# hkust-vgd/pointwise

Measured on AMD Instinct MI355X. Metric: conv3p fwd+bwd Mpoints/s, higher is better.
Workload: dtype f32; 1 GPU; cfg2 ModelNet40-shaped: B=32 clouds/GPU x N=2048, pointcnn2_acsd conv3p stack 3->9 s1, 9->9 s2, 9->9 s3, 9->9 s4 (+SELU), forward+backward, a different batch every step, next batch's neighbour search enqueued on a side stream under the current backward; global_batch=32, points_per_cloud=2048, parallelism=dp1, backward_kernel_choice=hint from Conv3pStack.tune() at set-up: short lists

## Files before the change

pointwise_amd/csrc/conv3p_abi_search.hpp:

```cpp
namespace {

template <typename T> int run_prep(const T *points, const Call<T> &c)
{
    if (c.skip_prep) {
        if (c.evicted_hinted)
            return hipMemsetAsync(c.L.slot[c.slot].cursor, 0, sizeof(uint32_t) * 2 * (size_t)c.d.B, c.s) == hipSuccess
                       ? CONV3P_OK : CONV3P_ERR_LAUNCH;
        return CONV3P_OK;
    }
    const Dims &d = c.d;
    Scope sc(K_PREP, c.s);
    if (d.N <= 16384 && d.N > kTile) {
        int npad = 128;
        while (npad < d.N) npad <<= 1;
        const int threads = npad / 2 < 1024 ? (npad / 2 < 64 ? 64 : npad / 2) : 1024;
        const size_t lds = (size_t)npad * 8 + 256;
        auto launch = [&](auto kern) {
            launch_lds(kern, dim3(d.B), dim3(threads), lds, c.s, points, d.N, d.ntiles, npad, c.L.pts, c.L.boxes, c.cc);
        };
        switch (npad / threads) {
        case 2: launch(prep_sort_kernel<T, 2>); break;
        case 4: launch(prep_sort_kernel<T, 4>); break;
        case 8: launch(prep_sort_kernel<T, 8>); break;
        default: launch(prep_sort_kernel<T, 16>); break;
        }
        return hip_ok();
    }
    dim3 grid((d.ntiles + kWavesPerBlock - 1) / kWavesPerBlock, d.B);
    hipLaunchKernelGGL(prep_kernel<T>, grid, dim3(256), 0, c.s, points, d.N, d.ntiles, c.L.pts, c.L.boxes, c.cc);
    return hip_ok();
}

template <typename T> size_t search_lds_bytes(const Stencil<T> &st, int gtiles)
{
    return lds_common(st) + a16((size_t)st.ntap * kCntStride * 4) + a16(sizeof(CentreRec<T>) * 64) + 64 * 3 * 4 +
           a16((size_t)gtiles * 64 * 8) + a16((size_t)gtiles * 4) + 32 + kWavesPerBlock * 64 * 4 +
           a16((size_t)kWavesPerBlock * 192 * 4) + a16((size_t)kWavesPerBlock * 256 * 4) + 1024;
}

template <typename T> int run_cloud_min(const T *points, const Call<T> &c)
{
    if (!c.st.window) return CONV3P_OK;
    hipLaunchKernelGGL(cloud_min_kernel<T>, dim3((unsigned)c.d.B), dim3(256), 0, c.s, points, c.d.N, c.L.cmin);
    return hip_ok();
}

template <typename SlotT> inline const uint32_t *sched_of(const SlotT &S)
{
#ifdef CONV3P_DEV_NO_SCHED
    return nullptr;
#else
    return S.sched;
#endif
}

constexpr unsigned long long kShortListsPerPoint = 35, kShortListsPerPointFused = 48;
template <typename T> SchedJob make_sched_job(const Call<T> &c, int slot, bool fused)
{
    const auto &S = c.L.slot[slot];
    return SchedJob{S.segs, S.sched, S.cursor, S.regime,
                    (fused ? kShortListsPerPointFused : kShortListsPerPoint) * (unsigned long long)c.d.B * (unsigned long long)c.d.N};
}

#ifndef CONV3P_DEV_FUSED_M
#define CONV3P_DEV_FUSED_M 6
#endif
template <typename T> bool fused_ok(const Call<T> &c)
{
#ifdef CONV3P_DEV_NO_FUSED_SEARCH
    return false;
#endif
    const Stencil<T> &st = c.st;
    if (c.L.ftab == nullptr || st.window) return false;
    for (int a = 0; a < 3; ++a)
        if (st.ext[a] > kFMaxExt) return false;
    return true;
}
template <typename T> FusedJob<T> make_fused_job(const Call<T> &c)
{
    const auto &S = c.L.slot[c.slot];
    FusedJob<T> j;
    j.st = c.st;
    j.cc = c.cc;
    j.count = S.count;
    j.tcount = S.tcount;
    j.pairs = S.pairs;
    j.segs = S.segs;
    j.qsegs = S.qsegs;
    j.qbm = S.qbm;
    j.qbm_hi = S.qbm_hi;
    for (int a = 0; a < 3; ++a)
        for (int k = 0; k < kFMaxExt; ++k)
            j.clo[a][k] = (float)(((double)k * c.st.step[a] - (double)c.st.full[a] * 0.5) * (double)kFR);
    return j;
}
inline int fused_mask_depth(int elem, int ntiles, int ntap_max, int maxfull_max)
{
    const int mmax = (ntiles + kWavesPerBlock - 1) / kWavesPerBlock;
    int M = std::min(mmax, (int)CONV3P_DEV_FUSED_M);
    if (ntiles <= 32) M = 1;
    if (M < 1) M = 1;
    while (M > 1 && fused_lds(ntap_max, maxfull_max, elem, M).total > 40 * 1024) --M;
    return fused_lds(ntap_max, maxfull_max, elem, M).total > kMaxLds ? 0 : M;
}
template <typename T> int launch_fused(const Call<T> &c, const FusedJobs<T> &jobs, const SchedJobs &sjobs, int njobs, bool schedule = true)
{
    const Dims &d = c.d;
    const BlockMap bm = make_blockmap(d);
    int ntap_max = 1, maxfull_max = 1;
    for (int k = 0; k < njobs; ++k) {
        ntap_max = std::max(ntap_max, jobs.job[k].st.ntap);
        maxfull_max = std::max(maxfull_max, jobs.job[k].st.maxfull);
    }
    const int M = fused_mask_depth((int)sizeof(T), d.ntiles, ntap_max, maxfull_max);
    if (M == 0) return CONV3P_ERR_UNSUPPORTED;
#ifdef CONV3P_DEV_FUSED_LDS_KB
    const size_t lds = std::max(fused_lds(ntap_max, maxfull_max, (int)sizeof(T), M).total, (size_t)CONV3P_DEV_FUSED_LDS_KB * 1024);
#else
    const size_t lds = fused_lds(ntap_max, maxfull_max, (int)sizeof(T), M).total;
#endif
    if (lds > kMaxLds) return CONV3P_ERR_UNSUPPORTED;
    const float inv16 = (float)((double)kFR / (double)c.st.voxel);
    Scope sc(K_SEARCH, c.s);
    hipLaunchKernelGGL(tile_tables_kernel<T>, dim3((d.ntiles + kWavesPerBlock - 1) / kWavesPerBlock, d.B), dim3(256), 0, c.s,
                       c.L.pts, d.ntiles, inv16, c.L.ftab, c.cc.version, c.L.tab_version, c.L.tab_ticket, c.L.tab_inv, c.cc.force);
    bool ext3 = true;
    for (int k = 0; k < njobs; ++k)
        for (int a = 0; a < 3; ++a) ext3 &= jobs.job[k].st.ext[a] == 3;
    auto launch = [&](auto kern) {
        launch_lds(kern, dim3(grid_of(bm), njobs), dim3(256), lds, c.s, c.L.pts, c.L.boxes, c.L.ftab, d.N, d.ntiles, c.L.ngroups, bm,
                   jobs, M, inv16);
    };
    if (ext3) launch(search_fused_kernel<T, true>);
    else launch(search_fused_kernel<T, false>);
#ifndef CONV3P_DEV_NO_SCHED
    if (schedule)
        hipLaunchKernelGGL(tile_sched_kernel, dim3(8, njobs), dim3(1024), 0, c.s, sjobs, d.B, d.ntiles, c.L.ngroups, bm.rounds * d.ntiles);
#endif
    return hip_ok();
}

template <typename T> int add_companions(const Call<T> &c, FusedJobs<T> &fj, SchedJobs &sj, int n)
{
    if (c.cache_key == nullptr || c.skip_prep) return n;
    const CacheRef ref = find_cache(c.cache_key);
    if (!ref) return n;
    CacheHost &h = *ref;
    for (int sl = 0; sl < h.nslots && n < kFusedMaxJobs; ++sl) {
        if (sl == c.slot || h.tags[sl] == 0ull) continue;
        const CacheHost::SlotDesc &sd = h.desc[sl];
        if (sd.voxel != (double)c.st.voxel) continue;
        Dims d2 = c.d;
        d2.fz = sd.fz; d2.fy = sd.fy; d2.fx = sd.fx;
        d2.ntap = sd.fz * sd.fy * sd.fx;
        Call<T> c2;
        c2.d = d2;
        c2.st = make_stencil<T>(d2, sd.stride, c.st.voxel);
        c2.L = c.L;
        c2.slot = sl;
        c2.s = c.s;
        c2.cc = make_ctl(c.L, sl, h.tags[sl], c.cc.epoch, 0);
        if (!fused_ok(c2)) continue;
        if (fused_mask_depth((int)sizeof(T), c.d.ntiles, std::max(c.st.ntap, c2.st.ntap), std::max(c.st.maxfull, c2.st.maxfull)) <
            fused_mask_depth((int)sizeof(T), c.d.ntiles, c.st.ntap, c.st.maxfull))
            continue;
        fj.job[n] = make_fused_job(c2);
        sj.job[n] = make_sched_job(c, sl, true);
        ++n;
    }
    return n;
}
template <typename T> void note_companions_built(const Call<T> &c, const FusedJobs<T> &fj, int n)
{
    if (c.cache_key == nullptr || n <= 1) return;
    const CacheRef ref = find_cache(c.cache_key);
    if (!ref) return;
    CacheHost &h = *ref;
    for (int k = 1; k < n; ++k)
        for (int sl = 0; sl < h.nslots; ++sl)
            if (sl != c.slot && h.tags[sl] == fj.job[k].cc.tag) h.built_gen[sl] = h.gen;
}

template <typename T> int run_search(const Call<T> &c, int32_t *count, bool with_pairs)
{
    if (c.skip_search && with_pairs) return CONV3P_OK;
    const Dims &d = c.d;
    const Stencil<T> &st = c.st;
    const auto &S = c.L.slot[c.slot];
    if (fused_ok(c) && fused_mask_depth((int)sizeof(T), d.ntiles, st.ntap, st.maxfull) > 0 && (!with_pairs || count == S.count)) {
        FusedJobs<T> fj;
        SchedJobs sj;
        fj.job[0] = make_fused_job(c);
        sj.job[0] = make_sched_job(c, c.slot, true);
        if (!with_pairs) {
            FusedJob<T> &j = fj.job[0];
            j.count = count;
            j.tcount = nullptr;
            j.pairs = nullptr;
            j.segs = nullptr;
            j.qsegs = nullptr;
            j.qbm = nullptr;
            j.qbm_hi = nullptr;
            return launch_fused<T>(c, fj, sj, 1, false);
        }
        const int nj = add_companions<T>(c, fj, sj, 1);
        TRY(launch_fused<T>(c, fj, sj, nj));
        note_companions_built<T>(c, fj, nj);
        return CONV3P_OK;
    }
    const size_t lds = search_lds_bytes(st, c.L.gtiles);
    if (lds > kMaxLds) return CONV3P_ERR_UNSUPPORTED;
    const BlockMap bm = make_blockmap(d);
    {
        Scope sc(K_SEARCH, c.s);
        auto launch = [&](auto kern, const T *cmin) {
            launch_lds(kern, dim3(grid_of(bm)), dim3(256), lds, c.s, c.L.pts, c.L.boxes, st, d.N, d.ntiles, c.L.gtiles, c.L.ngroups,
                       bm, count, with_pairs ? S.pairs : nullptr, c.cc, S.segs, S.qsegs, cmin, with_pairs ? S.tcount : nullptr,
                       with_pairs ? S.qbm : nullptr, with_pairs ? S.qbm_hi : nullptr);
        };
        if (st.window) launch(search_kernel<T, true>, c.L.cmin);
        else launch(search_kernel<T, false>, static_cast<const T *>(nullptr));
        if (with_pairs) {
            SchedJobs sj;
            sj.job[0] = make_sched_job(c, c.slot, false);
            hipLaunchKernelGGL(tile_sched_kernel, dim3(8, 1), dim3(1024), 0, c.s, sj, d.B, d.ntiles, c.L.ngroups, bm.rounds * d.ntiles);
        }
    }
    return hip_ok();
}

template <typename T> int run_geometry(const T *points, const Call<T> &c)
{
    TRY(run_prep<T>(points, c));
    TRY(run_cloud_min<T>(points, c));
    return run_search<T>(c, c.L.slot[c.slot].count, true);
}

#ifdef CONV3P_DEV_WALK_STATS
__global__ void walk_stats_kernel(const uint2 *qsegs, const PairEntry *pairs, int ntiles_all, unsigned long long *out)
{
    const int t = blockIdx.x * blockDim.x + threadIdx.x;
    if (t >= ntiles_all) return;
    uint32_t len[64];
    unsigned long long recs = 0, live = 0;
    for (int c = 0; c < 64; ++c) {
        const uint2 sg = qsegs[(size_t)t * 64 + c];
        len[c] = sg.y == kSegOverflow ? 0u : sg.y;
        recs += len[c];
        for (uint32_t i = 0; i < len[c]; ++i) live += code_fwd(pairs[sg.x + i].code) != kNoTap ? 1u : 0u;
    }
    unsigned long long cur = 0, pslw = 0, ideal = 0, curmax = 0, pslmax = 0, idealmax = 0;
    for (int w = 0; w < 4; ++w) {
        uint32_t mx = 0, sum = 0;
        for (int c = 0; c < 16; ++c) { mx = max(mx, len[16 * w + c]); sum += len[16 * w + c]; }
        const unsigned long long a = (mx + 3) / 4;
        uint32_t S = max(1u, (sum + 63) / 64);
        for (;; ++S) {
            uint32_t need = 0;
            for (int c = 0; c < 16; ++c) need += (len[16 * w + c] + S - 1) / S;
            if (need <= 64) break;
        }
        const unsigned long long idl = (sum + 63) / 64;
        cur += a; pslw += S; ideal += idl;
        curmax = max(curmax, a); pslmax = max(pslmax, (unsigned long long)S); idealmax = max(idealmax, idl);
    }
    uint32_t St = max(1u, (uint32_t)((recs + 255) / 256));
    for (;; ++St) {
        uint32_t need = 0;
        for (int c = 0; c < 64; ++c) need += (len[c] + St - 1) / St;
        if (need <= 256) break;
    }
    atomicAdd(&out[0], recs); atomicAdd(&out[1], live); atomicAdd(&out[2], cur); atomicAdd(&out[3], pslw);
    atomicAdd(&out[4], 4ull * St); atomicAdd(&out[5], ideal);
    atomicMax(&out[6], curmax); atomicMax(&out[7], pslmax); atomicMax(&out[8], (unsigned long long)St); atomicMax(&out[9], idealmax);
}
template <typename T> void dev_walk_stats(const Call<T> &c, const char *what, int ci, int co)
{
    const auto &S = c.L.slot[c.slot];
    if (c.L.ngroups != 1) return;
    unsigned long long *d = nullptr, h[10];
    if (hipMalloc(&d, sizeof(h)) != hipSuccess) return;
    (void)hipMemsetAsync(d, 0, sizeof(h), c.s);
    const int nt = c.d.B * c.d.ntiles;
    hipLaunchKernelGGL(walk_stats_kernel, dim3((nt + 63) / 64), dim3(64), 0, c.s, S.qsegs, S.pairs, nt, d);
    (void)hipStreamSynchronize(c.s);
    (void)hipMemcpy(h, d, sizeof(h), hipMemcpyDeviceToHost);
    (void)hipFree(d);
    const double r = (double)h[0];
    fprintf(stderr, "walk_stats %s<%d,%d> stride %d B=%d N=%d: records/point %.2f (true pairs %.2f) | lane use: shipped %.3f (true-pair %.3f), "
            "per-wave proportional %.3f, per-workgroup proportional %.3f, bound %.3f | steps of the slowest wave: shipped %llu, "
            "per-wave prop. %llu, per-wg prop. %llu, bound %llu | mean steps per wave: %.2f / %.2f / %.2f / %.2f\n",
            what, ci, co, c.st.step[0], c.d.B, c.d.N, r / ((double)c.d.B * c.d.N), (double)h[1] / ((double)c.d.B * c.d.N),
            r / (64.0 * h[2]), (double)h[1] / (64.0 * h[2]), r / (64.0 * h[3]), r / (64.0 * h[4]), r / (64.0 * h[5]),
            h[6], h[7], h[8], h[9], h[2] / (4.0 * nt), h[3] / (4.0 * nt), h[4] / (4.0 * nt), h[5] / (4.0 * nt));
}
#endif

template <typename T>
int prepare_multi_impl(const T *points, const int32_t *strides, int K, T voxel, int B, int N, int fz, int fy,
                       int fx, Where wh, void *stream)
{
    if (K <= 0 || K > kMaxJobs || !strides) return CONV3P_ERR_INVALID_ARGUMENT;
    Dims d{B, N, 0, 0, fz, fy, fx, 0, 0};
    for (int k = 0; k < K; ++k) TRY(check(d, strides + 3 * k, (double)voxel, false));
    if ((size_t)B * N == 0) return CONV3P_OK;
    if (!points) return CONV3P_ERR_INVALID_ARGUMENT;
    if (K > wh.nslots) return CONV3P_ERR_WORKSPACE;
    hipStream_t s = static_cast<hipStream_t>(stream);
    SearchJobs<T> jobs;
    FusedJobs<T> fjobs;
    SchedJobs sjobs, fsjobs;
    int njobs = 0, nfused = 0;
    size_t lds = 0;
    bool any_window = false;
    Call<T> c;
    for (int k = 0; k < K; ++k) {
        TRY(begin_call<T>(c, d, strides + 3 * k, voxel, 0, wh, s));
        TRY(run_prep<T>(points, c));
        wh.flags |= CONV3P_CACHE_POINTS_UNCHANGED;
        if (c.skip_search) continue;
        const Stencil<T> &st = c.st;
        const auto &S = c.L.slot[c.slot];
        TRY(run_cloud_min<T>(points, c));
        if (fused_ok(c) && fused_mask_depth((int)sizeof(T), c.d.ntiles, c.st.ntap, c.st.maxfull) > 0) {
            fjobs.job[nfused] = make_fused_job(c);
            fsjobs.job[nfused++] = make_sched_job(c, c.slot, true);
            continue;
        }
        any_window |= st.window != 0;
        const size_t l = search_lds_bytes(st, c.L.gtiles);
        if (l > kMaxLds) return CONV3P_ERR_UNSUPPORTED;
        lds = l > lds ? l : lds;
        SearchJob<T> &j = jobs.job[njobs++];
        j.st = st;
        j.cc = c.cc;
        j.count = S.count;
        j.tcount = S.tcount;
        j.pairs = S.pairs;
        j.segs = S.segs;
        j.qsegs = S.qsegs;
        j.qbm = S.qbm;
        j.qbm_hi = S.qbm_hi;
        sjobs.job[njobs - 1] = make_sched_job(c, c.slot, true);
    }
    if (nfused > 0) TRY(launch_fused<T>(c, fjobs, fsjobs, nfused));
    if (njobs == 0) return CONV3P_OK;
    for (int k = 0; k < njobs; ++k)
        sjobs.job[k].limit = kShortListsPerPoint * (unsigned long long)c.d.B * (unsigned long long)c.d.N;
#ifndef CONV3P_DEV_JOBS_IN_ORDER
    for (int a = 1; a < njobs; ++a)
        for (int b2 = a; b2 > 0; --b2) {
            auto vol = [](const SearchJob<T> &j) { return (long long)j.st.step[0] * j.st.step[1] * j.st.step[2]; };
            if (vol(jobs.job[b2]) <= vol(jobs.job[b2 - 1])) break;
            std::swap(jobs.job[b2], jobs.job[b2 - 1]);
            std::swap(sjobs.job[b2], sjobs.job[b2 - 1]);
        }
#endif
    const BlockMap bm = make_blockmap(c.d);
    {
        Scope sc(K_SEARCH, s);
        auto launch = [&](auto kern) {
            launch_lds(kern, dim3(grid_of(bm), njobs), dim3(256), lds, s, c.L.pts, c.L.boxes, c.d.N, c.d.ntiles, c.L.gtiles,
                       c.L.ngroups, bm, jobs, c.L.cmin);
        };
        if (any_window) launch(search_multi_kernel<T, true>);
        else launch(search_multi_kernel<T, false>);
        hipLaunchKernelGGL(tile_sched_kernel, dim3(8, njobs), dim3(1024), 0, s, sjobs, c.d.B, c.d.ntiles, c.L.ngroups,
                           bm.rounds * c.d.ntiles);
    }
    return hip_ok();
}

}
```

pointwise_amd/csrc/conv3p_search_fused.hpp:

```cpp
#pragma once

#include "conv3p_device.hpp"

namespace conv3p {

constexpr int kFR = 16;
constexpr int kFK = 96;
constexpr int kFEntries = 116;
constexpr int kFHeader = 3 * kFEntries;
constexpr int kFTableU64 = kFHeader + 4;
constexpr int kFMaxExt = 8;
#ifndef CONV3P_DEV_FUSED_ABLATE
#define CONV3P_DEV_FUSED_ABLATE 0
#endif
constexpr int kFStream = 192;
constexpr int kFMaxE = 12;

__device__ __forceinline__ int floor_i32(float x)
{
    int r;
    asm("v_cvt_flr_i32_f32_e32 %0, %1" : "=v"(r) : "v"(x));
    return r;
}
__device__ __forceinline__ bool finite3(float x, float y, float z)
{
    return (x - x) + (y - y) + (z - z) == 0.0f;
}

template <typename T>
__global__ __launch_bounds__(256) void tile_tables_kernel(const PointRec<T> *__restrict__ pts, int ntiles, float inv16,
                                                          unsigned long long *__restrict__ tables,
                                                          const uint32_t *__restrict__ version,
                                                          uint32_t *__restrict__ tab_version,
                                                          uint32_t *__restrict__ tab_ticket,
                                                          uint32_t *__restrict__ tab_inv,
                                                          int force)
{
    __shared__ __attribute__((aligned(16))) unsigned long long tab[kWavesPerBlock][kFTableU64];
    const int wave = threadIdx.x >> 6, lane = threadIdx.x & 63;
    const int tile = blockIdx.x * kWavesPerBlock + wave;
    const int b = blockIdx.y;
    if (tile >= ntiles) return;
    if (!force && tab_version[b] == version[b] && tab_inv[b] == __builtin_bit_cast(uint32_t, inv16)) return;
    const size_t t = (size_t)b * ntiles + tile;
    const PointRec<T> r = pts[t * kTile + lane];
    const float v[3] = {(float)r.x, (float)r.y, (float)r.z};
    const bool valid = r.idx >= 0 && finite3(v[0], v[1], v[2]);
    float tmin[3], ext = 0.0f;
#pragma unroll
    for (int a = 0; a < 3; ++a) {
        tmin[a] = wave_min(valid ? v[a] : __builtin_huge_valf());
        const float tmax = wave_max(valid ? v[a] : -__builtin_huge_valf());
        ext = fmaxf(ext, (tmax - tmin[a]) * inv16);
    }
    const uint64_t allv = __ballot(valid);
    int e = 0;
    if (allv == 0) {
        tmin[0] = tmin[1] = tmin[2] = 0.0f;
    } else if (!(ext < 1.0e30f)) {
        e = kFMaxE + 1;
    } else {
        while (e <= kFMaxE && floor_i32(ext) >> e > kFK - 1) ++e;
    }
    const int es = e > 31 ? 31 : e;
    const int ws = (kFR >> es) + 2;
    int beta[3];
#pragma unroll
    for (int a = 0; a < 3; ++a) {
        int b16 = floor_i32((v[a] - tmin[a]) * inv16) >> es;
        b16 = b16 < 0 ? 0 : (b16 > kFK - 1 ? kFK - 1 : b16);
        beta[a] = b16;
    }
    unsigned long long *mytab = tab[wave];
    {
        uint4 *z = reinterpret_cast<uint4 *>(mytab);
        for (int i = lane; i < kFTableU64 / 2; i += 64) z[i] = make_uint4(0, 0, 0, 0);
    }
    __builtin_amdgcn_wave_barrier();
    if (valid) {
        const unsigned long long bit = 1ull << lane;
        for (int i = 1; i <= ws; ++i) {
#pragma unroll
            for (int a = 0; a < 3; ++a) atomicOr(&mytab[a * kFEntries + beta[a] + i], bit);
        }
    }
    __builtin_amdgcn_wave_barrier();
    if (lane == 0) {
        mytab[kFHeader + 0] = (uint64_t)__builtin_bit_cast(uint32_t, tmin[0]) | ((uint64_t)__builtin_bit_cast(uint32_t, tmin[1]) << 32);
        mytab[kFHeader + 1] = (uint64_t)__builtin_bit_cast(uint32_t, tmin[2]) | ((uint64_t)(uint32_t)e << 32);
        mytab[kFHeader + 2] = allv;
        mytab[kFHeader + 3] = 0;
    }
    __builtin_amdgcn_wave_barrier();
    __builtin_amdgcn_s_waitcnt(0xc07f);
    const uint4 *src = reinterpret_cast<const uint4 *>(mytab);
    uint4 *dst = reinterpret_cast<uint4 *>(tables + t * kFTableU64);
    for (int i = lane; i < kFTableU64 / 2; i += 64) dst[i] = src[i];
    if (!force && lane == 0) {
        const uint32_t done = atomicAdd(&tab_ticket[b], 1u);
        if (done + 1u == (uint32_t)ntiles) {
            tab_inv[b] = __builtin_bit_cast(uint32_t, inv16);
            tab_version[b] = version[b];
            tab_ticket[b] = 0;
        }
    }
}

template <typename T> struct FusedJob {
    Stencil<T> st;
    CacheCtl cc;
    int32_t *count, *tcount;
    PairEntry *pairs;
    uint2 *segs, *qsegs;
    uint32_t *qbm, *qbm_hi;
    float clo[3][kFMaxExt];
};
constexpr int kFusedMaxJobs = 8;
template <typename T> struct FusedJobs {
    FusedJob<T> job[kFusedMaxJobs];
};

struct FusedLds {
    size_t tapmap, cnt, cen, bmk, nqw, misc, red, tab, masks, stream, total;
};
__host__ __device__ inline size_t f_a16(size_t x) { return (x + 15) & ~(size_t)15; }
__host__ __device__ inline FusedLds fused_lds(int ntap, int maxfull, int elem, int M)
{
    FusedLds L;
    size_t off = 0;
    L.tapmap = off; off += f_a16((size_t)3 * maxfull * 2);
    L.cnt = off; off += f_a16((size_t)ntap * kCntStride * 4);
    L.cen = off; off += (size_t)64 * 12 * elem;
    L.bmk = off; off += (ntap > 64 ? 256 : ntap > 32 ? 128 : 64) * 4;
    L.nqw = off; off += (size_t)kWavesPerBlock * 64 * 4;
    L.misc = off; off += 16;
    L.red = off; off += 6 * 8;
    off = f_a16(off);
    L.tab = off; off += (size_t)kWavesPerBlock * kFTableU64 * 8;
    L.masks = off; off += (size_t)kWavesPerBlock * M * 64 * 8;
    L.stream = off; off += (size_t)kWavesPerBlock * 2 * kFStream * 4;
    L.total = off;
    return L;
}

template <typename T>
__device__ __forceinline__ uint64_t tiles_meeting(const T *__restrict__ cloud_box, int ntiles, int base, const T *ulo, const T *uhi)
{
    const int t = base + (threadIdx.x & 63);
    bool ov = false;
    if (t < ntiles) {
        const T *bb = cloud_box + (size_t)t * 6;
        const T b0 = bb[0], b1 = bb[1], b2 = bb[2], b3 = bb[3], b4 = bb[4], b5 = bb[5];
        ov = !((b3 < ulo[0]) | (b0 > uhi[0]) | (b4 < ulo[1]) | (b1 > uhi[1]) | (b5 < ulo[2]) | (b2 > uhi[2]));
    }
    return __ballot(ov);
}

template <typename T>
__device__ __forceinline__ uint64_t fused_mask(const FusedJob<T> &job, const unsigned long long *tab, const float *gs, int e)
{
    uint64_t H = ~0ull;
#pragma unroll
    for (int a = 0; a < 3; ++a) {
        uint64_t A = 0;
        const unsigned long long *ta = tab + a * kFEntries;
        for (int k = 0; k < job.st.ext[a]; ++k) {
            int j = floor_i32(gs[a] + job.clo[a][k]) >> e;
            j = j < 0 ? 0 : (j > kFEntries - 1 ? kFEntries - 1 : j);
            A |= ta[j];
        }
        H &= A;
    }
    return H;
}

template <typename T> struct TapFast {
    static constexpr bool enabled = false;
};
template <> struct TapFast<float> {
    static constexpr bool enabled = true;
};
__device__ __forceinline__ float min3_t(float a, float b, float c) { return fminf(fminf(a, b), c); }
__device__ __forceinline__ double min3_t(double a, double b, double c) { return fmin(fmin(a, b), c); }
__device__ __forceinline__ int clamp_tap(int t, int full)
{
    t = t > full - 1 ? full - 1 : t;
    return t < 0 ? 0 : t;
}

template <typename T> struct __attribute__((aligned(16))) CenRec {
    T lo[3], hi[3], p[3];
    T pad[3];
};

template <typename T>
__device__ __forceinline__ void fused_resolve(const Stencil<T> &st, T rvoxel, const int16_t *tapmap, uint32_t *cnt, uint32_t *bmk,
                                              const CenRec<T> *cen, uint32_t ql, const PointRec<T> &v, bool on, bool want_bwd,
                                              bool want_bm, uint32_t &fwd, uint32_t &bwd)
{
    const CenRec<T> c = cen[ql];
    const T d[3] = {v.x - c.lo[0], v.y - c.lo[1], v.z - c.lo[2]};
    const T dm = min3_t(d[0], d[1], d[2]);
    const T em = min3_t(c.hi[0] - v.x, c.hi[1] - v.y, c.hi[2] - v.z);
    const bool in = on && dm >= (T)0 && em >= (T)0;
    const T vv[3] = {v.x, v.y, v.z};
    fwd = kNoTap;
    bwd = kNoTap;
    bool exact = in;
    if (TapFast<T>::enabled) {
        int t[3];
        bool near = false;
#pragma unroll
        for (int a = 0; a < 3; ++a) {
            const float q = (float)d[a] * (float)rvoxel;
            const float mag = fmaxf(fabsf((float)c.p[a]), fabsf((float)vv[a]));
            near |= fabsf(q - __builtin_rintf(q)) <= __builtin_fmaf(mag, 5.0e-7f * (float)rvoxel, 1.0e-6f * (float)st.full[a]);
            t[a] = (int)q;
        }
        exact = in && near;
        if (in && !near) {
            const int tx = tapmap[clamp_tap(t[0], st.full[0])];
            const int ty = tapmap[st.maxfull + clamp_tap(t[1], st.full[1])];
            const int tz = tapmap[2 * st.maxfull + clamp_tap(t[2], st.full[2])];
            if ((tx | ty | tz) >= 0) {
                fwd = (uint32_t)((tz * st.ext[1] + ty) * st.ext[0] + tx);
                bwd = (uint32_t)st.ntap - 1u - fwd;
            }
        }
    }
    if (exact) {
        const int tx = tapmap[clamp_tap((int)(d[0] / st.voxel), st.full[0])];
        const int ty = tapmap[st.maxfull + clamp_tap((int)(d[1] / st.voxel), st.full[1])];
        const int tz = tapmap[2 * st.maxfull + clamp_tap((int)(d[2] / st.voxel), st.full[2])];
        if ((tx | ty | tz) >= 0) {
            fwd = (uint32_t)((tz * st.ext[1] + ty) * st.ext[0] + tx);
            if (want_bwd) {
                const T lx = (T)((double)v.x - st.half[0]), ly = (T)((double)v.y - st.half[1]), lz = (T)((double)v.z - st.half[2]);
                const int bx = tapmap[clamp_tap((int)((c.p[0] - lx) / st.voxel), st.full[0])];
                const int by = tapmap[st.maxfull + clamp_tap((int)((c.p[1] - ly) / st.voxel), st.full[1])];
                const int bz = tapmap[2 * st.maxfull + clamp_tap((int)((c.p[2] - lz) / st.voxel), st.full[2])];
                if ((bx | by | bz) >= 0) bwd = (uint32_t)((bz * st.ext[1] + by) * st.ext[0] + bx);
            }
        }
    }
    if (fwd != kNoTap) {
        atomicAdd(&cnt[fwd * kCntStride + ql], 1u);
        if (want_bm && bwd != kNoTap) atomicOr(&bmk[ql + ((bwd >> 5) << 6)], 1u << (bwd & 31u));
    }
}

typedef int int4_a4 __attribute__((ext_vector_type(4), aligned(4)));

template <typename T> __device__ __forceinline__ bool fused_compacts(const Stencil<T> &st, uint32_t tile_hits)
{
    return !(CONV3P_DEV_FUSED_ABLATE & 16) && (st.step[0] * st.step[1] * st.step[2] > 1 || tile_hits > 48u * 64u);
}

template <typename T, bool EXT3>
__global__ __launch_bounds__(256) void search_fused_kernel(const PointRec<T> *__restrict__ pts, const T *__restrict__ boxes,
                                                           const unsigned long long *__restrict__ tables, int N, int ntiles,
                                                           int ngroups, BlockMap bm, FusedJobs<T> jobs, int M, float inv16)
{
    extern __shared__ __attribute__((aligned(16))) char smem[];
    const int wave = threadIdx.x >> 6, lane = threadIdx.x & 63;
    int b, qt;
    if (!block_to_cloud(bm, b, qt)) return;
    const FusedJob<T> &job = jobs.job[blockIdx.y];
    const bool have_pairs = job.pairs != nullptr;
    if (have_pairs && slot_valid(job.cc, b)) return;
    const Stencil<T> &st = job.st;

    const FusedLds L = fused_lds(st.ntap, st.maxfull, (int)sizeof(T), M);
    int16_t *tapmap = reinterpret_cast<int16_t *>(smem + L.tapmap);
    uint32_t *cnt = reinterpret_cast<uint32_t *>(smem + L.cnt);
    CenRec<T> *cen = reinterpret_cast<CenRec<T> *>(smem + L.cen);
    uint32_t *bmk = reinterpret_cast<uint32_t *>(smem + L.bmk);
    uint32_t *nqw = reinterpret_cast<uint32_t *>(smem + L.nqw);
    uint32_t *misc = reinterpret_cast<uint32_t *>(smem + L.misc);
    T *red = reinterpret_cast<T *>(smem + L.red);
    unsigned long long *tab = reinterpret_cast<unsigned long long *>(smem + L.tab) + (size_t)wave * kFTableU64;
    unsigned long long *masks = reinterpret_cast<unsigned long long *>(smem + L.masks) + (size_t)wave * M * 64;

    const PointRec<T> *cloud_pts = pts + (size_t)b * ntiles * kTile;
    const T *cloud_box = boxes + (size_t)b * ntiles * 6;
    const unsigned long long *cloud_tab = tables + (size_t)b * ntiles * kFTableU64;
    const PointRec<T> me = cloud_pts[(size_t)qt * kTile + lane];
    const float pf[3] = {(float)me.x, (float)me.y, (float)me.z};
    const bool qvalid = me.idx >= 0 && finite3(pf[0], pf[1], pf[2]);
    const bool want_bm = job.qbm != nullptr && (st.ntap <= 32 || (st.ntap <= 128 && job.qbm_hi != nullptr));

    build_tapmap(tapmap, st.full, st.step, st.maxfull);
    for (int e = threadIdx.x; e < st.ntap * kCntStride; e += blockDim.x) cnt[e] = 0;
    if (wave == 0) {
        CenRec<T> r;
        const T p[3] = {me.x, me.y, me.z};
#pragma unroll
        for (int a = 0; a < 3; ++a) {
            r.lo[a] = (T)((double)p[a] - st.half[a]);
            r.hi[a] = (T)((double)p[a] + st.half[a]);
            r.p[a] = p[a];
            r.pad[a] = (T)0;
        }
        cen[lane] = r;
        bmk[lane] = 0;
        if (st.ntap > 32) bmk[64 + lane] = 0;
        if (st.ntap > 64) bmk[128 + lane] = bmk[192 + lane] = 0;
    } else {
        const int a = wave - 1;
        const T pa = a == 0 ? me.x : (a == 1 ? me.y : me.z);
        const T mn = wave_min(qvalid ? pa : Limits<T>::inf()), mx = wave_max(qvalid ? pa : -Limits<T>::inf());
        if (lane == 0) {
            red[a] = mn;
            red[3 + a] = mx;
        }
    }
    const float q0[3] = {1.0e-3f + 4.0e-6f * (fabsf(pf[0]) * inv16), 1.0e-3f + 4.0e-6f * (fabsf(pf[1]) * inv16),
                         1.0e-3f + 4.0e-6f * (fabsf(pf[2]) * inv16)};
    __syncthreads();
    T ulo[3], uhi[3];
#pragma unroll
    for (int a = 0; a < 3; ++a) {
        ulo[a] = (T)((double)red[a] - st.half[a]);
        uhi[a] = (T)((double)red[3 + a] + st.half[a]);
    }
    const float s16[3] = {(float)(kFR * st.step[0]), (float)(kFR * st.step[1]), (float)(kFR * st.step[2])};

    auto for_my_tiles = [&](auto &&visit) {
        for (int base = 0; base < ntiles; base += 64) {
            uint64_t todo = tiles_meeting(cloud_box, ntiles, base, ulo, uhi) & (0x1111111111111111ull << wave);
            while (todo) {
                const int i = __builtin_ctzll(todo);
                todo &= todo - 1;
                visit(base + i, todo ? base + __builtin_ctzll(todo) : -1);
            }
        }
    };
    uint4 pf0 = make_uint4(0, 0, 0, 0), pf1 = pf0, pf2 = pf0;
    int pf_ct = -1;
    auto request = [&](int ct) {
        const uint4 *src = reinterpret_cast<const uint4 *>(cloud_tab + (size_t)ct * kFTableU64);
        pf0 = src[lane];
        pf1 = src[64 + lane];
        pf2 = src[128 + (lane < kFTableU64 / 2 - 128 ? lane : 0)];
        pf_ct = ct;
    };
    auto compute_mask = [&](int ct, int nxt) -> uint64_t {
        if (pf_ct != ct) request(ct);
        uint4 *dst = reinterpret_cast<uint4 *>(tab);
        __builtin_amdgcn_wave_barrier();
        dst[lane] = pf0;
        dst[64 + lane] = pf1;
        if (lane < kFTableU64 / 2 - 128) dst[128 + lane] = pf2;
        __builtin_amdgcn_wave_barrier();
        if (nxt >= 0) request(nxt);
        if (CONV3P_DEV_FUSED_ABLATE & 4) return 0ull;
        const uint64_t h0 = tab[kFHeader], h1 = tab[kFHeader + 1];
        const float tmin[3] = {__builtin_bit_cast(float, (uint32_t)h0), __builtin_bit_cast(float, (uint32_t)(h0 >> 32)),
                               __builtin_bit_cast(float, (uint32_t)h1)};
        const int e = (int)(uint32_t)(h1 >> 32);
        const int es = e > kFMaxE ? kFMaxE : e;
        const int ws = (kFR >> es) + 2;
        float gs[3], smax = 0.0f;
#pragma unroll
        for (int a = 0; a < 3; ++a) {
            const float g = (pf[a] - tmin[a]) * inv16;
            const float slack = __builtin_fmaf(4.0e-6f, fabsf(g), q0[a]);
            smax = fmaxf(smax, slack);
            gs[a] = (g - slack) + (float)(ws << es);
        }
        const bool wide = e > kFMaxE || __any(qvalid && !(smax <= 0.2f * (float)(1 << es)));
        auto entry = [&](float x) {
            int j = floor_i32(x) >> es;
            return j < 0 ? 0 : (j > kFEntries - 1 ? kFEntries - 1 : j);
        };
        uint64_t h;
        if (wide) {
            h = tab[kFHeader + 2];
        } else if (EXT3) {
            uint64_t A[3];
#pragma unroll
            for (int a = 0; a < 3; ++a) {
                const float x1 = gs[a] - (float)(kFR / 2);
                const unsigned long long *ta = tab + a * kFEntries;
                const uint64_t r0 = ta[entry(x1 - s16[a])], r1 = ta[entry(x1)], r2 = ta[entry(x1 + s16[a])];
                A[a] = r0 | r1 | r2;
            }
            h = A[0] & A[1] & A[2];
        } else {
            h = fused_mask(job, tab, gs, es);
        }
        return qvalid ? h : 0ull;
    };

    {
        uint32_t mine = 0;
        int ord = 0;
        for_my_tiles([&](int ct, int nxt) {
            const uint64_t m = compute_mask(ct, nxt);
            mine += (uint32_t)__popcll(m);
            if (ord < M) masks[(size_t)ord * 64 + lane] = m;
            ++ord;
        });
        nqw[wave * 64 + lane] = mine;
    }
    __syncthreads();

    if (wave == 0) {
        const uint32_t n0 = nqw[lane], n1 = nqw[64 + lane], n2 = nqw[128 + lane], n3 = nqw[192 + lane];
        const uint32_t nq = n0 + n1 + n2 + n3;
        int Ltot;
        const uint32_t offq = (uint32_t)wave_excl_scan((int)nq, Ltot);
        const uint32_t cap = job.cc.pairs_per_cloud;
        uint32_t base = 0, ok = 0;
        if (!have_pairs) {
            if (lane == 0) misc[0] = misc[1] = misc[2] = 0;
        } else {
        if (lane == 0) {
            base = Ltot ? atomicAdd(&job.cc.cursor[b], (uint32_t)Ltot) : 0u;
            ok = (base <= cap && (uint32_t)Ltot <= cap - base) ? 1u : 0u;
            if (!ok) atomicSub(&job.cc.cursor[b], (uint32_t)Ltot);
            base += (uint32_t)b * cap;
            job.segs[((size_t)b * ntiles + qt) * ngroups] = ok ? make_uint2(base, (uint32_t)Ltot) : make_uint2(0u, kSegOverflow);
            for (int g = 1; g < ngroups; ++g) job.segs[((size_t)b * ntiles + qt) * ngroups + g] = make_uint2(0u, 0u);
            misc[0] = base;
            misc[1] = ok;
            misc[2] = (uint32_t)Ltot;
        }
        base = __shfl(base, 0);
        ok = __shfl(ok, 0);
        if (!ok || !fused_compacts(st, (uint32_t)Ltot))
            job.qsegs[((size_t)b * ntiles + qt) * ngroups * 64 + lane] = ok ? make_uint2(base + offq, nq) : make_uint2(0u, kSegOverflow);
        for (int g = 1; g < ngroups; ++g) job.qsegs[(((size_t)b * ntiles + qt) * ngroups + g) * 64 + lane] = make_uint2(0u, 0u);
        }
        nqw[lane] = offq;
        nqw[64 + lane] = offq + n0;
        nqw[128 + lane] = offq + n0 + n1;
        nqw[192 + lane] = offq + n0 + n1 + n2;
    }
    __syncthreads();
    const bool ok = misc[1] != 0;
    const uint32_t gbase = misc[0];
    char *pbase = reinterpret_cast<char *>(job.pairs + gbase);
    const T rvoxel = (T)1 / st.voxel;

    if (!(CONV3P_DEV_FUSED_ABLATE & 2)) {
        uint32_t *sdesc = reinterpret_cast<uint32_t *>(smem + L.stream) + wave * (2 * kFStream);
        uint32_t *sslot = sdesc + kFStream;
        uint32_t off = nqw[wave * 64 + lane] * 8u;
        int have = 0, ord = 0;
        pf_ct = -1;
        auto drain = [&](int n) {
            if (CONV3P_DEV_FUSED_ABLATE & 1) return;
            constexpr int kU = 2;
            uint32_t d[kU], so[kU];
            PointRec<T> v[kU];
#pragma unroll
            for (int u = 0; u < kU; ++u) {
                const int i = u * 64 + lane;
                d[u] = sdesc[i < n ? i : 0];
                so[u] = sslot[i < n ? i : 0];
            }
#pragma unroll
            for (int u = 0; u < kU; ++u) v[u] = cloud_pts[(size_t)((d[u] >> 12) * kTile + (d[u] & 63u))];
#pragma unroll
            for (int u = 0; u < kU; ++u) {
                const bool on = u * 64 + lane < n;
                const uint32_t ql = (d[u] >> 6) & 63u;
                uint32_t fwd, bwd;
                fused_resolve<T>(st, rvoxel, tapmap, cnt, bmk, cen, ql, v[u], on, true, want_bm, fwd, bwd);
                if (on && ok) {
                    PairEntry pe;
                    pe.cand = (uint32_t)v[u].idx;
                    pe.code = pair_code(fwd, bwd, ql);
                    *reinterpret_cast<PairEntry *>(pbase + so[u]) = pe;
                }
            }
        };
        for_my_tiles([&](int ct, int nxt) {
            uint64_t mm = ord < M ? masks[(size_t)ord * 64 + lane] : compute_mask(ct, nxt);
            ++ord;
            const uint32_t dbase = ((uint32_t)ct << 12) | ((uint32_t)lane << 6);
            while (true) {
                const uint64_t act = __ballot(mm != 0);
                if (act == 0) break;
                if (mm != 0) {
                    const uint32_t c = (uint32_t)__builtin_ctzll(mm);
                    mm &= mm - 1;
                    const int at = have + (int)__builtin_amdgcn_mbcnt_hi((uint32_t)(act >> 32), __builtin_amdgcn_mbcnt_lo((uint32_t)act, 0));
                    sdesc[at] = dbase | c;
                    sslot[at] = off;
                    off += 8u;
                }
                have += __popcll(act);
                __builtin_amdgcn_wave_barrier();
                if (have >= 128) {
                    drain(128);
                    __builtin_amdgcn_wave_barrier();
                    const uint32_t cd = sdesc[128 + lane], cs = sslot[128 + lane];
                    __builtin_amdgcn_wave_barrier();
                    sdesc[lane] = cd;
                    sslot[lane] = cs;
                    have -= 128;
                    __builtin_amdgcn_wave_barrier();
                }
            }
        });
        if (have > 0) drain(have);
    }
    __threadfence_block();
    __syncthreads();

    if (have_pairs && ok && fused_compacts(st, misc[2])) {
        uint32_t *livec = nqw + 64;
        {
            const int c = wave * 16 + (lane & 15);
            uint32_t sacc = 0;
            for (int f = lane >> 4; f < st.ntap; f += 4) sacc += cnt[f * kCntStride + c];
            sacc += lane_xor16(sacc);
            sacc += lane_xor32(sacc);
            if (lane < 16) livec[c] = sacc;
        }
        __builtin_amdgcn_wave_barrier();
        const uint32_t r0 = nqw[wave * 16], r1 = wave == kWavesPerBlock - 1 ? misc[2] : nqw[wave * 16 + 16];
        PairEntry *tp = job.pairs + gbase;
        const uint64_t lt = lane == 0 ? 0ull : (~0ull >> (64 - lane));
        uint32_t carry = 0;
        constexpr int kCB = 4;
        PairEntry cur[kCB], nxt[kCB];
        auto request = [&](PairEntry (&dst)[kCB], uint32_t pos) {
#pragma unroll
            for (int u = 0; u < kCB; ++u) {
                const uint32_t i = pos + (uint32_t)(u * 64 + lane);
                dst[u] = tp[i < r1 ? i : r0];
            }
        };
        if (r0 < r1) request(nxt, r0);
        for (uint32_t pos = r0; pos < r1; pos += 64 * kCB) {
#pragma unroll
            for (int u = 0; u < kCB; ++u) cur[u] = nxt[u];
            if (pos + 64 * kCB < r1) request(nxt, pos + 64 * kCB);
#pragma unroll
            for (int u = 0; u < kCB; ++u) {
                const uint32_t cpos = pos + (uint32_t)(u * 64);
                if (cpos >= r1) break;
                const uint32_t i = cpos + (uint32_t)lane;
                const bool valid = i < r1;
                const uint32_t c = code_q(cur[u].code) & 63u;
                const bool live = valid && code_fwd(cur[u].code) != kNoTap;
                const uint32_t oc = nqw[c], lv = livec[c];
                const uint64_t Lm = __ballot(live);
                const uint32_t sc = oc > cpos ? oc - cpos : 0u;
                const uint64_t before = Lm & lt & ~((1ull << (sc & 63u)) - 1ull);
                const uint32_t rank = (uint32_t)__popcll(before) + (oc < cpos ? carry : 0u);
                if (live && oc + rank != i) tp[oc + rank] = cur[u];
                if (valid && i - oc >= lv) {
                    PairEntry dead;
                    dead.cand = cur[u].cand;
                    dead.code = pair_code(kNoTap, kNoTap, c);
                    tp[i] = dead;
                }
                carry = (uint32_t)__builtin_amdgcn_readlane((int)(rank + (live ? 1u : 0u)), 63);
            }
        }
        if (lane < 16) {
            const int c = wave * 16 + lane;
            job.qsegs[((size_t)b * ntiles + qt) * ngroups * 64 + c] = make_uint2(gbase + nqw[c], livec[c]);
        }
    }

    if (!(CONV3P_DEV_FUSED_ABLATE & 8)) {
        if (job.count != nullptr && me.idx >= 0) {
            int32_t *row = job.count + ((size_t)b * N + me.idx) * st.ntap;
            const int pieces = st.ntap >> 2;
            for (int pc = wave; pc < pieces; pc += kWavesPerBlock) {
                const uint32_t *src = cnt + (size_t)(pc * 4) * kCntStride + lane;
                int4_a4 w;
                w.x = (int)src[0];
                w.y = (int)src[kCntStride];
                w.z = (int)src[2 * kCntStride];
                w.w = (int)src[3 * kCntStride];
                *reinterpret_cast<int4_a4 *>(row + pc * 4) = w;
            }
            if (wave == (pieces & 3))
                for (int f = pieces * 4; f < st.ntap; ++f) row[f] = (int32_t)cnt[f * kCntStride + lane];
        }
        if (job.tcount != nullptr) {
            int32_t *tc = job.tcount + ((size_t)b * ntiles + qt) * st.ntap * kTile;
            for (int f = wave; f < st.ntap; f += kWavesPerBlock) tc[f * kTile + lane] = (int32_t)cnt[f * kCntStride + lane];
        }
        if (want_bm && wave == 0) {
            job.qbm[((size_t)b * ntiles + qt) * 64 + lane] = bmk[lane];
            if (st.ntap > 32) job.qbm_hi[((size_t)b * ntiles + qt) * 64 + lane] = bmk[64 + lane];
            if (st.ntap > 64) {
                const size_t pstride = (size_t)(job.qbm_hi - job.qbm);
                job.qbm_hi[pstride + ((size_t)b * ntiles + qt) * 64 + lane] = bmk[128 + lane];
                job.qbm_hi[2 * pstride + ((size_t)b * ntiles + qt) * 64 + lane] = bmk[192 + lane];
            }
        }
    }
    __syncthreads();
    if (threadIdx.x == 0 && have_pairs) {
        const CacheCtl &cc = job.cc;
        const uint32_t t = atomicAdd(&cc.ticket[b], 1u);
        if (t + 1u == (uint32_t)bm.blocks_per_cloud) {
            cc.built_version[b] = cc.version[b];
            cc.built_tag[b] = cc.tag;
            cc.ticket[b] = 0;
        }
    }
}

}
```

Measured before the change: 165.5 Mpoints/s.

## Narrow fused search window by one bin with slack-aware fallback lookups

Shrinks the per-tile bit-table window from (R>>e)+2 to (R>>e)+1 bins, so fewer false-positive candidate points pass the fused mask. To keep correctness near bin edges, the query computes a second bin index offset by the slack and ORs in extra table rows when any lane lands in a different bin. Tap lookups now use integer offsets instead of float adds. The compaction threshold and short-list budget are retuned to 40 hits per point, and the stride-only compaction trigger is dropped. The extra wave-uniform branches and lookups add cost on edge cases, and the tighter window risks missed neighbours if the slack bound is wrong.

```diff
diff --git a/pointwise_amd/csrc/conv3p_abi_search.hpp b/pointwise_amd/csrc/conv3p_abi_search.hpp
--- a/pointwise_amd/csrc/conv3p_abi_search.hpp
+++ b/pointwise_amd/csrc/conv3p_abi_search.hpp
@@ -54,7 +54,7 @@
 #endif
 }
 
-constexpr unsigned long long kShortListsPerPoint = 35, kShortListsPerPointFused = 48;
+constexpr unsigned long long kShortListsPerPoint = 35, kShortListsPerPointFused = kFHitsOf32Neighbours;
 template <typename T> SchedJob make_sched_job(const Call<T> &c, int slot, bool fused)
 {
     const auto &S = c.L.slot[slot];
diff --git a/pointwise_amd/csrc/conv3p_search_fused.hpp b/pointwise_amd/csrc/conv3p_search_fused.hpp
--- a/pointwise_amd/csrc/conv3p_search_fused.hpp
+++ b/pointwise_amd/csrc/conv3p_search_fused.hpp
@@ -27,6 +27,9 @@
     return (x - x) + (y - y) + (z - z) == 0.0f;
 }
 
+__host__ __device__ constexpr int fused_window(int es) { return (kFR >> es) >= 1 ? (kFR >> es) + 1 : 2; }
+static_assert(kFEntries >= kFK + fused_window(0) + 1 && kFEntries % 2 == 0, "window entries per axis");
+
 template <typename T>
 __global__ __launch_bounds__(256) void tile_tables_kernel(const PointRec<T> *__restrict__ pts, int ntiles, float inv16,
                                                           unsigned long long *__restrict__ tables,
@@ -63,7 +66,7 @@
         while (e <= kFMaxE && floor_i32(ext) >> e > kFK - 1) ++e;
     }
     const int es = e > 31 ? 31 : e;
-    const int ws = (kFR >> es) + 2;
+    const int ws = fused_window(es);
     int beta[3];
 #pragma unroll
     for (int a = 0; a < 3; ++a) {
@@ -157,7 +160,8 @@
 }
 
 template <typename T>
-__device__ __forceinline__ uint64_t fused_mask(const FusedJob<T> &job, const unsigned long long *tab, const float *gs, int e)
+__device__ __forceinline__ uint64_t fused_mask(const FusedJob<T> &job, const unsigned long long *tab, const float *gs, const float *fz,
+                                               bool qvalid, int e)
 {
     uint64_t H = ~0ull;
 #pragma unroll
@@ -165,9 +169,12 @@
         uint64_t A = 0;
         const unsigned long long *ta = tab + a * kFEntries;
         for (int k = 0; k < job.st.ext[a]; ++k) {
-            int j = floor_i32(gs[a] + job.clo[a][k]) >> e;
+            const float x = gs[a] + job.clo[a][k];
+            int j = floor_i32(x) >> e, jh = floor_i32(x + fz[a]) >> e;
             j = j < 0 ? 0 : (j > kFEntries - 1 ? kFEntries - 1 : j);
+            jh = jh < 0 ? 0 : (jh > kFEntries - 1 ? kFEntries - 1 : jh);
             A |= ta[j];
+            if (__any(qvalid && jh != j)) A |= ta[jh];
         }
         H &= A;
     }
@@ -251,9 +258,10 @@
 
 typedef int int4_a4 __attribute__((ext_vector_type(4), aligned(4)));
 
+constexpr uint32_t kFHitsOf32Neighbours = 40;
 template <typename T> __device__ __forceinline__ bool fused_compacts(const Stencil<T> &st, uint32_t tile_hits)
 {
-    return !(CONV3P_DEV_FUSED_ABLATE & 16) && (st.step[0] * st.step[1] * st.step[2] > 1 || tile_hits > 48u * 64u);
+    return !(CONV3P_DEV_FUSED_ABLATE & 16) && tile_hits > kFHitsOf32Neighbours * 64u;
 }
 
 template <typename T, bool EXT3>
@@ -323,7 +331,7 @@
         ulo[a] = (T)((double)red[a] - st.half[a]);
         uhi[a] = (T)((double)red[3 + a] + st.half[a]);
     }
-    const float s16[3] = {(float)(kFR * st.step[0]), (float)(kFR * st.step[1]), (float)(kFR * st.step[2])};
+    const int S16[3] = {kFR * st.step[0], kFR * st.step[1], kFR * st.step[2]};
 
     auto for_my_tiles = [&](auto &&visit) {
         for (int base = 0; base < ntiles; base += 64) {
@@ -359,18 +367,19 @@
                                __builtin_bit_cast(float, (uint32_t)h1)};
         const int e = (int)(uint32_t)(h1 >> 32);
         const int es = e > kFMaxE ? kFMaxE : e;
-        const int ws = (kFR >> es) + 2;
-        float gs[3], smax = 0.0f;
+        const int ws = fused_window(es);
+        float gs[3], fz[3], smax = 0.0f;
 #pragma unroll
         for (int a = 0; a < 3; ++a) {
             const float g = (pf[a] - tmin[a]) * inv16;
             const float slack = __builtin_fmaf(4.0e-6f, fabsf(g), q0[a]);
             smax = fmaxf(smax, slack);
             gs[a] = (g - slack) + (float)(ws << es);
+            fz[a] = 2.5f * slack;
         }
         const bool wide = e > kFMaxE || __any(qvalid && !(smax <= 0.2f * (float)(1 << es)));
-        auto entry = [&](float x) {
-            int j = floor_i32(x) >> es;
+        auto entry = [&](int i, int d) {
+            const int j = (int)((uint32_t)i + (uint32_t)d) >> es;
             return j < 0 ? 0 : (j > kFEntries - 1 ? kFEntries - 1 : j);
         };
         uint64_t h;
@@ -378,16 +387,30 @@
             h = tab[kFHeader + 2];
         } else if (EXT3) {
             uint64_t A[3];
+            int ih[3];
+            bool far[3];
 #pragma unroll
             for (int a = 0; a < 3; ++a) {
                 const float x1 = gs[a] - (float)(kFR / 2);
+                const int i1 = floor_i32(x1);
+                ih[a] = floor_i32(x1 + fz[a]);
+                far[a] = ((i1 ^ ih[a]) >> es) != 0;
                 const unsigned long long *ta = tab + a * kFEntries;
-                const uint64_t r0 = ta[entry(x1 - s16[a])], r1 = ta[entry(x1)], r2 = ta[entry(x1 + s16[a])];
+                const uint64_t r0 = ta[entry(i1, -S16[a])], r1 = ta[entry(i1, 0)], r2 = ta[entry(i1, S16[a])];
                 A[a] = r0 | r1 | r2;
+            }
+            if (__any(qvalid && (far[0] | far[1] | far[2]))) {
+#pragma unroll
+                for (int a = 0; a < 3; ++a) {
+                    if (!__any(qvalid && far[a])) continue;
+                    const unsigned long long *ta = tab + a * kFEntries;
+                    const uint64_t r0 = ta[entry(ih[a], -S16[a])], r1 = ta[entry(ih[a], 0)], r2 = ta[entry(ih[a], S16[a])];
+                    A[a] |= r0 | r1 | r2;
+                }
             }
             h = A[0] & A[1] & A[2];
         } else {
-            h = fused_mask(job, tab, gs, es);
+            h = fused_mask(job, tab, gs, fz, qvalid, es);
         }
         return qvalid ? h : 0ull;
     };
```

New measurement: 172.2 Mpoints/s (median of 6 runs). 1.04x the previous value.
